# summa-dev/halo2-experiments

Hardware: AMD Instinct MI355X
Metric: BN256 G1 MSM throughput (higher is better)
Workload: dtype u32; 1 GPU; standalone BN256 G1 MSM, 2^24 points per GPU (global 2^24 x 1; BASELINE configs[4] microbench, north-star headline size); points_per_gpu=16777216, global_points=16777216, base_set=fixed-base table (registration default from 2^17 points), window_bits=22, windows=12, parallelism=index-range shards x1, all-gather of 96 B partials (RCCL) + host fold, base_set_bytes=12901679104

## Files before the change

halo2-experiments_amd/csrc/g1.h:

```cpp
#pragma once
#include "ff29.h"

namespace hm {

using Fq = Fe<FqParams>;
using Fr = Fe<FrParams>;

struct G1Aff {
  Fq x, y;
};
struct G1Jac {
  Fq x, y, z;
  bool inf;
};

#define HM_G1_XB 12.0
#define HM_G1_YB 5.0
#define HM_G1_ZB 2.0

#ifdef HM_BOUNDS
inline void g1_check_class(const G1Jac& p, const char* what) {
  HM_CHECK(p.x.lb <= MASK29 && p.y.lb <= MASK29 && p.z.lb <= MASK29, what);
  HM_CHECK(p.x.vb <= HM_G1_XB && p.y.vb <= HM_G1_YB && p.z.vb <= HM_G1_ZB, what);
}
// ... 202 lines not shown
  } else {
    u2 = fe_mul(q.x, acc.zz);
  }
  const Fq pp0 = fe_norm(fe_sub<9, 29>(u2, acc.x));
  if constexpr (!LOCKSTEP) {
    pp = fe_sqr(pp0);
    if (fe_is_zero_mod(pp)) return false;
    s2p = fe_mul(q.y, acc.zzz);
  }
  Fq s2;
  {
    const Fq s2n = fe_sub<3, 29>(fe_zero<FqParams>(), s2p);
#pragma unroll
    for (int i = 0; i < 9; ++i) s2.l[i] = neg ? s2n.l[i] : s2p.l[i];
#ifdef HM_BOUNDS
    s2.vb = s2n.vb; s2.lb = s2n.lb; s2.tb = s2n.tb;
#endif
  }
  const Fq r = fe_norm(fe_sub<4, 29>(s2, acc.y));
  if constexpr (LOCKSTEP) {
    fe_sqr_x2(pp, rr, pp0, r);
    if (fe_is_zero_mod(pp)) return false;
    fe_mul_x3(ppp, qq, zz3, pp0, pp, acc.x, pp, acc.zz, pp);
  } else {
    ppp = fe_mul(pp0, pp);
    qq = fe_mul(acc.x, pp);
    rr = fe_sqr(r);
  }
  const Fq t2 = fe_add(ppp, fe_dbl(qq));
  const Fq x3 = fe_norm(fe_sub<6, 31>(rr, t2));
  const Fq vx = fe_sub<9, 29>(qq, x3);
  const Fq ny = fe_sub<4, 29>(fe_zero<FqParams>(), acc.y);
  if constexpr (LOCKSTEP) {
    fe_mul_mul2(zzz3, y3, acc.zzz, ppp, r, vx, ny, ppp);
  } else {
    y3 = fe_mul2(r, vx, ny, ppp);
    zz3 = fe_mul(acc.zz, pp);
    zzz3 = fe_mul(acc.zzz, ppp);
  }
  acc.x = x3;
  acc.y = y3;
  acc.zz = zz3;
  acc.zzz = zzz3;
  return true;
}

HM_HD G1Xyzz g1x_madd(const G1Xyzz& p, const G1Aff& q, bool neg = false) {
  if (p.inf) return g1x_from_affine(neg ? g1_neg_affine(q) : q);
  G1Xyzz r = p;
  if (g1x_madd_fast(r, q, neg)) return r;
  return g1x_from_jac(g1_madd_nz(g1x_to_jac(p), q, neg));
}

}
```

halo2-experiments_amd/csrc/host_check.cpp:

```cpp
#include <algorithm>
#include <cstring>
#include <utility>
#include <vector>

#include "g1.h"
#include "graph_lower.h"
#include "host_fr.h"
#include "mock_check.h"

namespace hm {
#include "g1_codec.inc"
#include "verify_read.inc"
#include "verify_terms.inc"
#include "poseidon.inc"
#include "range.inc"
#include "keygen.inc"
#include "shplonk.inc"
#include "pairing.inc"
#include "transcript.inc"
}

using namespace hm;

namespace {
// ... 173 lines not shown
}
void hc_g1_double(const uint64_t* pj, int pinf, uint64_t* out, int* out_inf) {
  store_jac(out, out_inf, g1_double(load_jac(pj, pinf)));
}
void hc_g1_chain(const uint64_t* q_aff, int k, int dbl, uint64_t* out, int* out_inf) {
  G1Aff q;
  q.x = load_ext<FqParams>(q_aff);
  q.y = load_ext<FqParams>(q_aff + 4);
  G1Jac acc = g1_identity();
  for (int i = 0; i < k; ++i) acc = g1_madd(acc, q);
  for (int i = 0; i < dbl; ++i) acc = g1_double(acc);
  store_jac(out, out_inf, acc);
}

void hc_g1x_chain(const uint64_t* q_affs, int k, uint64_t signs, uint64_t* out, int* out_inf) {
  G1Xyzz acc = g1x_identity();
  for (int i = 0; i < k; ++i) {
    G1Aff q;
    q.x = load_ext<FqParams>(q_affs + 8 * i);
    q.y = load_ext<FqParams>(q_affs + 8 * i + 4);
    acc = g1x_madd(acc, q, ((signs >> (i & 63)) & 1) != 0);
  }
  store_jac(out, out_inf, g1x_to_jac(acc));
}

int hc_xyzz_bounds_closure(const uint64_t* pj, const uint64_t* q_aff, double* report) {
  G1Jac pjac = load_jac(pj, 0);
  G1Xyzz p = g1x_from_jac(pjac);
  force_bounds(p.x, HM_XYZZ_XB);
  force_bounds(p.y, HM_XYZZ_YB);
  force_bounds(p.zz, 2.0);
  force_bounds(p.zzz, 2.0);
  G1Aff q;
  q.x = load_ext<FqParams>(q_aff);
  q.y = load_ext<FqParams>(q_aff + 4);
  force_bounds(q.x, 2.0);
  force_bounds(q.y, 2.0);
  G1Xyzz r = p;
  if (!g1x_madd_fast(r, q, true)) return 0;
  {
    G1Xyzz rl = p;
    if (!g1x_madd_fast<true>(rl, q, true)) return 0;
    for (int i = 0; i < 9; ++i)
      if (rl.x.l[i] != r.x.l[i] || rl.y.l[i] != r.y.l[i] || rl.zz.l[i] != r.zz.l[i] || rl.zzz.l[i] != r.zzz.l[i]) return 0;
    if (rl.x.vb > HM_XYZZ_XB || rl.y.vb > HM_XYZZ_YB || rl.zz.vb > 2.0 || rl.zzz.vb > 2.0) return 0;
  }
  const G1Jac j = g1x_to_jac(p);
  report[0] = r.x.vb; report[1] = r.y.vb; report[2] = r.zz.vb; report[3] = r.zzz.vb;
  report[4] = j.x.vb; report[5] = j.y.vb; report[6] = j.z.vb;
  int ok = 1;
  if (r.x.vb > HM_XYZZ_XB || r.y.vb > HM_XYZZ_YB || r.zz.vb > 2.0 || r.zzz.vb > 2.0) ok = 0;
  if (j.x.vb > HM_G1_XB || j.y.vb > HM_G1_YB || j.z.vb > HM_G1_ZB) ok = 0;
  return ok;
}

int hc_bounds_closure(const uint64_t* pj, const uint64_t* qj, const uint64_t* q_aff, double* report) {
  G1Jac p = load_jac(pj, 0), q2 = load_jac(qj, 0);
  at_class_max(p);
  at_class_max(q2);
  G1Aff q;
  q.x = load_ext<FqParams>(q_aff);
  q.y = load_ext<FqParams>(q_aff + 4);
  force_bounds(q.x, 2.0);
  force_bounds(q.y, 2.0);
  G1Jac r[3] = {g1_madd_nz(p, q, true), g1_add_nz(p, q2), g1_double_nz(p)};
  int ok = 1;
  for (int i = 0; i < 3; ++i) {
    report[3 * i + 0] = r[i].x.vb;
    report[3 * i + 1] = r[i].y.vb;
    report[3 * i + 2] = r[i].z.vb;
    if (r[i].x.vb > HM_G1_XB || r[i].y.vb > HM_G1_YB || r[i].z.vb > HM_G1_ZB) ok = 0;
    if (r[i].x.lb > MASK29 || r[i].y.lb > MASK29 || r[i].z.lb > MASK29) ok = 0;
  }
  return ok;
}

int hc_graph_bounds_closure(const uint64_t* a_ext, double* report) {
  typedef Fe<FrParams> F;
  F x = load_ext<FrParams>(a_ext);
  const double CAP = 16.0;
  int ok = 1, r = 0;
  F c16 = x, c16b = x, c3 = x, col = x;
  force_bounds(c16, CAP);
  force_bounds(c16b, CAP);
  force_bounds(c3, 3.0);
  force_bounds(col, 6.0);
  F m = fe_mul(c16, c16b);
  report[r++] = m.vb;
  ok &= m.vb <= 3.0;
  F q = fe_sqr(c16);
  ok &= q.vb <= 3.0;
  ok &= fe_mul(col, c16).vb <= 3.0;
  F h8 = x;
  force_bounds(h8, 8.0);
  F s16 = fe_norm(fe_add(h8, h8));
  report[r++] = s16.vb;
  ok &= s16.vb <= CAP;
  F red = fe_reduce_small(fe_norm(fe_add(c16, c16b)));
  ok &= red.vb <= 3.0;
  F dbl = fe_reduce_small(fe_norm(fe_dbl(c16)));
  ok &= dbl.vb <= 3.0;
  F d12 = x;
  force_bounds(d12, 12.0);
  F sub_lazy = fe_norm(fe_sub<4, 29>(d12, c3));
  report[r++] = sub_lazy.vb;
  ok &= sub_lazy.vb <= CAP;
// ... 641 lines not shown
```

halo2-experiments_amd/csrc/msm.hip:

```cpp
#include <hip/hip_runtime.h>

#include <algorithm>
#include <chrono>
#include <cmath>
#include <cstdlib>

#include "hm_internal.h"
#include "host_fq.h"
#include "host_fr.h"
#include "msm_dev.h"

namespace hm {


__global__ void msm_init_counters_kernel(uint32_t* __restrict__ bcnt, size_t nbt, uint32_t* __restrict__ br_count,
                                         uint32_t* __restrict__ khist, uint32_t nkeys, uint32_t* __restrict__ big_count) {
  const size_t i0 = (size_t)blockIdx.x * blockDim.x + threadIdx.x, stride = (size_t)gridDim.x * blockDim.x;
  for (size_t i = i0; i < nbt; i += stride) bcnt[i] = 0;
  if (i0 < nkeys) khist[i0] = 0;
  if (i0 < 4) {
    if (br_count) br_count[i0] = 0;
    big_count[i0] = 0;
  }
}
// ... 1069 lines not shown
    if (rem) {
      const uint32_t key = task_key(rem, L);
      task_bucket[t0 + full] = b;
      task_order[base[key] + atomicAdd(&h[key], 1u)] = t0 + full;
    }
  }
  __syncthreads();
  const uint32_t nh = hot_n < ORDER_HOT ? hot_n : ORDER_HOT;
  for (uint32_t e = 0; e < nh; ++e) {
    const uint32_t b = hot[e][0], t0 = hot[e][1], full = hot[e][2], at = hot[e][3];
    for (uint32_t i = threadIdx.x; i < full; i += ORDER_THREADS) {
      task_bucket[t0 + i] = b;
      task_order[at + i] = t0 + i;
    }
  }
}

#ifndef HM_K3_WAVES
#define HM_K3_WAVES 4
#endif
#define HM_K3_OCC __attribute__((amdgpu_waves_per_eu(HM_K3_WAVES, HM_K3_WAVES)))
__global__ __launch_bounds__(ACC_THREADS) HM_K3_OCC void msm_accumulate_kernel(const uint32_t* __restrict__ sorted,
                                                                     const uint32_t* __restrict__ task_bucket,
                                                                     const uint32_t* __restrict__ task_order,
                                                                     const uint32_t* __restrict__ boff,
                                                                     const uint32_t* __restrict__ bcnt,
                                                                     const uint32_t* __restrict__ toff,
                                                                     const uint32_t* __restrict__ xy,
                                                                     uint32_t* __restrict__ partial,
                                                                     const uint32_t* __restrict__ totals,
                                                                     const uint32_t* __restrict__ pairs, uint32_t L_host) {
  __shared__ uint4 stage[4][ACC_THREADS];
  const uint32_t L = effective_task_len(pairs, L_host);
  const uint32_t lane = threadIdx.x;
  const uint32_t slot = blockIdx.x * ACC_THREADS + lane;
  const uint32_t T = totals[1];
  uint32_t start = 0, end = 0, t = 0;
  if (slot < T) {
    t = task_order[slot];
    const uint32_t b = task_bucket[t];
    const uint32_t k = t - toff[b];
    start = boff[b] + k * L;
    const uint32_t bucket_end = boff[b] + bcnt[b];
    end = start + L < bucket_end ? start + L : bucket_end;
  }
  if (start >= end) return;
  const G1Jac res = accumulate_chain<true>(sorted, xy, start, end, stage, lane);
  store_jac(partial + (size_t)t * PT_WORDS, res);
}


constexpr uint32_t FINALIZE_SERIAL = 8;
constexpr uint32_t FINALIZE_SLICE = 2048;
__global__ __launch_bounds__(ACC_THREADS) void msm_bucket_finalize_kernel(const uint32_t* __restrict__ partial,
                                                                          const uint32_t* __restrict__ toff,
                                                                          uint32_t* __restrict__ bucket, uint32_t NBT,
                                                                          uint32_t* __restrict__ big_count,
                                                                          uint32_t* __restrict__ big_list,
                                                                          uint2* __restrict__ slice_list,
                                                                          const uint32_t* __restrict__ totals) {
  const uint32_t b = blockIdx.x * ACC_THREADS + threadIdx.x;
  if (b >= NBT) return;
  if (totals[2]) {
    store_jac(bucket + (size_t)b * PT_WORDS, g1_identity());
    return;
  }
  const uint32_t lo = toff[b], hi = toff[b + 1];
  if (hi - lo > FINALIZE_SERIAL) {
    big_list[atomicAdd(big_count, 1u)] = b;
    if (hi - lo > FINALIZE_SLICE) {
      const uint32_t nsl = (hi - lo + FINALIZE_SLICE - 1) / FINALIZE_SLICE;
      const uint32_t at = atomicAdd(big_count + 1, nsl);
      for (uint32_t k = 0; k < nsl; ++k) slice_list[at + k] = make_uint2(b, k);
    }
    return;
  }
  G1Jac acc = g1_identity();
  for (uint32_t t = lo; t < hi; ++t) acc = g1_add(acc, load_jac(partial + (size_t)t * PT_WORDS));
  store_jac(bucket + (size_t)b * PT_WORDS, acc);
}

__global__ __launch_bounds__(WIN_THREADS) void msm_bucket_finalize_slices_kernel(uint32_t* __restrict__ partial,
                                                                                 const uint32_t* __restrict__ toff,
                                                                                 const uint32_t* __restrict__ big_count,
                                                                                 const uint2* __restrict__ slice_list) {
  __shared__ uint32_t tree[WIN_THREADS * PT_WORDS];
  const uint32_t count = big_count[1];
  for (uint32_t item = blockIdx.x; item < count; item += gridDim.x) {
    const uint2 e = slice_list[item];
    const uint32_t lo = toff[e.x] + e.y * FINALIZE_SLICE;
    const uint32_t end = toff[e.x + 1], hi = lo + FINALIZE_SLICE < end ? lo + FINALIZE_SLICE : end;
    G1Jac acc = g1_identity();
    for (uint32_t t = lo + threadIdx.x; t < hi; t += WIN_THREADS) acc = g1_add(acc, load_jac(partial + (size_t)t * PT_WORDS));
    const G1Jac r = block_sum_points(tree, acc);
    if (threadIdx.x == 0) store_jac(partial + (size_t)lo * PT_WORDS, r);
    __syncthreads();
  }
}

__global__ __launch_bounds__(WIN_THREADS) void msm_bucket_finalize_big_kernel(const uint32_t* __restrict__ partial,
                                                                              const uint32_t* __restrict__ toff,
                                                                              uint32_t* __restrict__ bucket,
                                                                              const uint32_t* __restrict__ big_count,
                                                                              const uint32_t* __restrict__ big_list) {
  __shared__ uint32_t tree[WIN_THREADS * PT_WORDS];
  const uint32_t count = *big_count;
  for (uint32_t item = blockIdx.x; item < count; item += gridDim.x) {
    const uint32_t b = big_list[item];
    const uint32_t lo = toff[b], hi = toff[b + 1];
    const uint32_t step = hi - lo > FINALIZE_SLICE ? FINALIZE_SLICE : 1u;
    G1Jac acc = g1_identity();
    for (uint32_t t = lo + threadIdx.x * step; t < hi; t += WIN_THREADS * step)
      acc = g1_add(acc, load_jac(partial + (size_t)t * PT_WORDS));
    const G1Jac r = block_sum_points(tree, acc);
    if (threadIdx.x == 0) store_jac(bucket + (size_t)b * PT_WORDS, r);
    __syncthreads();
  }
}

__global__ __launch_bounds__(ACC_THREADS) void msm_reduce_segments_kernel(const uint32_t* __restrict__ bucket,
                                                                          uint32_t* __restrict__ segres, uint32_t W,
                                                                          uint32_t NB, uint32_t NBP, uint32_t SEG,
                                                                          uint32_t nseg) {
  const uint32_t idx = blockIdx.x * ACC_THREADS + threadIdx.x;
  if (idx >= W * nseg) return;
  const uint32_t w = idx / nseg, sgi = idx - w * nseg;
  const uint32_t lo = sgi * SEG + 1;
  const uint32_t hi = lo + SEG - 1 < NB ? lo + SEG - 1 : NB;
  const uint32_t* bw = bucket + (size_t)w * NBP * PT_WORDS;
  G1Jac run = g1_identity(), acc = g1_identity();
  G1Jac cur = hi >= lo ? load_jac(bw + (size_t)hi * PT_WORDS) : g1_identity();
  for (uint32_t b = hi; b >= lo; --b) {
    const G1Jac nxt = b > lo ? load_jac(bw + (size_t)(b - 1) * PT_WORDS) : g1_identity();
    run = g1_add(run, cur);
    acc = g1_add(acc, run);
    cur = nxt;
  }
  uint32_t m = lo - 1;
  if (m != 0 && !run.inf) {
    G1Jac r = g1_identity();
    for (int bit = 31 - __clz(m); bit >= 0; --bit) {
      r = g1_double(r);
      if ((m >> bit) & 1) r = g1_add(r, run);
    }
    acc = g1_add(acc, r);
  }
  store_jac(segres + (size_t)idx * PT_WORDS, acc);
}

#ifndef HM_SUM_PER_LANE
#define HM_SUM_PER_LANE 4
#endif
constexpr uint32_t SUM_SPAN = WIN_THREADS * HM_SUM_PER_LANE;
__global__ __launch_bounds__(WIN_THREADS) void msm_sum_points_kernel(const uint32_t* __restrict__ in, uint32_t count,
                                                                     uint32_t* __restrict__ out, uint32_t out_count) {
  __shared__ uint32_t tree[WIN_THREADS * PT_WORDS];
  const uint32_t w = blockIdx.y, blk = blockIdx.x, t = threadIdx.x;
  const uint32_t* sw = in + (size_t)w * count * PT_WORDS;
  const uint32_t lo = blk * SUM_SPAN, hi = lo + SUM_SPAN < count ? lo + SUM_SPAN : count;
  G1Jac acc = g1_identity();
  for (uint32_t s = lo + t; s < hi; s += WIN_THREADS) acc = g1_add(acc, load_jac(sw + (size_t)s * PT_WORDS));
  const G1Jac r = block_sum_points(tree, acc);
  if (t == 0) store_jac(out + ((size_t)w * out_count + blk) * PT_WORDS, r);
}

__global__ __launch_bounds__(WIN_THREADS) void msm_reduce_rowcol_kernel(const uint32_t* __restrict__ bucket, uint32_t* __restrict__ sums,
                                                                        uint32_t m, uint32_t h) {
  __shared__ uint32_t tree[WIN_THREADS * PT_WORDS];
  const uint32_t M = 1u << m, H = 1u << h, blk = blockIdx.x, t = threadIdx.x;
  bucket += (size_t)blockIdx.y * ((size_t)M * H + 1) * PT_WORDS;
  sums += (size_t)blockIdx.y * ((size_t)M + H) * PT_WORDS;
  const bool row = blk < H;
  const uint32_t count = row ? M : H;
  const uint32_t first = row ? blk * M : blk - H, stride = row ? 1u : M;
  const uint32_t* b1 = bucket + PT_WORDS;
  G1Jac acc = g1_identity();
  if (t < count) {
    G1Jac cur = load_jac(b1 + (size_t)(first + t * stride) * PT_WORDS);
    for (uint32_t e = t; e < count; e += WIN_THREADS) {
      const uint32_t en = e + WIN_THREADS;
      const G1Jac nxt = en < count ? load_jac(b1 + (size_t)(first + en * stride) * PT_WORDS) : g1_identity();
      acc = g1_add(acc, cur);
      cur = nxt;
    }
  }
  const G1Jac r = block_sum_points_upto(tree, acc, count < WIN_THREADS ? count : WIN_THREADS);
  if (t == 0) store_jac(sums + (size_t)blk * PT_WORDS, r);
}

__global__ __launch_bounds__(WIN_THREADS) void msm_reduce_bits_kernel(const uint32_t* __restrict__ sums, uint32_t m, uint32_t h,
                                                                      uint32_t* __restrict__ winres, uint32_t res_stride) {
  __shared__ uint32_t tree[WIN_THREADS * PT_WORDS];
  const uint32_t M = 1u << m, H = 1u << h, p = blockIdx.x, t = threadIdx.x;
  sums += (size_t)blockIdx.y * ((size_t)M + H) * PT_WORDS;
  if (blockIdx.y != 0 && p == 0 && t < 4) (winres - 4)[(size_t)blockIdx.y * res_stride + t] = (winres - 4)[t];
  winres += (size_t)blockIdx.y * res_stride;
  const uint32_t* rows = sums;
  const uint32_t* cols = sums + (size_t)H * PT_WORDS;
  G1Jac acc = g1_identity();
  uint32_t widest = 0;
  if (p < m) {
    const uint32_t half = M >> 1, low = (1u << p) - 1u;
    for (uint32_t i = t; i < half; i += WIN_THREADS) {
      const uint32_t lo = ((i & ~low) << 1) | (1u << p) | (i & low);
      acc = g1_add(acc, load_jac(cols + (size_t)lo * PT_WORDS));
    }
    widest = half;
    if (p == 0) {
      for (uint32_t hi = t; hi < H; hi += WIN_THREADS) acc = g1_add(acc, load_jac(rows + (size_t)hi * PT_WORDS));
      if (H > widest) widest = H;
    }
  } else {
    const uint32_t q = p - m, half = H >> 1, low = (1u << q) - 1u;
    for (uint32_t i = t; i < half; i += WIN_THREADS) {
      const uint32_t hi = ((i & ~low) << 1) | (1u << q) | (i & low);
      acc = g1_add(acc, load_jac(rows + (size_t)hi * PT_WORDS));
    }
    widest = half;
  }
  if (widest > WIN_THREADS) widest = WIN_THREADS;
  if (widest < 1) widest = 1;
  const G1Jac r = block_sum_points_upto(tree, acc, widest);
  if (t == 0) store_window_ext(winres + (size_t)p * 32, r);
}

__global__ void msm_windows_to_ext_kernel(const uint32_t* __restrict__ in, uint32_t W, uint32_t* __restrict__ winres) {
  const uint32_t w = blockIdx.x * blockDim.x + threadIdx.x;
  if (w >= W) return;
  store_window_ext(winres + (size_t)w * 32, load_jac(in + (size_t)w * PT_WORDS));
}

struct G1AffineWords {
  uint32_t w[16];
};
__global__ void g1_fixed_table_kernel(G1AffineWords base_ext, uint32_t* __restrict__ table) {
  const uint32_t w = blockIdx.x * blockDim.x + threadIdx.x;
  if (w >= 64) return;
  uint32_t wx[8], wy[8];
#pragma unroll
  for (int k = 0; k < 8; ++k) { wx[k] = base_ext.w[k]; wy[k] = base_ext.w[8 + k]; }
  G1Aff b;
  b.x = fe_from_ext<FqParams>(wx);
  b.y = fe_from_ext<FqParams>(wy);
  G1Jac p = g1_from_affine(b);
  for (uint32_t k = 0; k < 4 * w; ++k) p = g1_double(p);
  G1Jac acc = p;
  for (uint32_t d = 1; d <= 15; ++d) {
    store_jac(table + ((size_t)w * 15 + (d - 1)) * PT_WORDS, acc);
    acc = g1_add(acc, p);
  }
}

__device__ __forceinline__ Fq fq_inverse(const Fq& a) {
  uint32_t e[9];
#pragma unroll
  for (int i = 0; i < 9; ++i) e[i] = FqParams::MOD[i];
  e[0] -= 2;
  Fq acc = fe_one<FqParams>();
  for (int i = 8; i >= 0; --i) {
    const int top = i == 8 ? 24 : 28;
    for (int bit = top; bit >= 0; --bit) {
      acc = fe_sqr(acc);
      if ((e[i] >> bit) & 1) acc = fe_mul(acc, a);
    }
  }
  return acc;
}

__global__ __launch_bounds__(ACC_THREADS) void msm_precompute_kernel(uint32_t* __restrict__ table,
                                                                     const uint8_t* __restrict__ inf, size_t n, uint32_t c,
                                                                     uint32_t W, uint32_t n_wide) {
  const size_t i = (size_t)blockIdx.x * ACC_THREADS + threadIdx.x;
  if (i >= n) return;
  if (inf[i]) {
    for (uint32_t j = 1; j < W; ++j) {
      uint4* o = reinterpret_cast<uint4*>(table + ((size_t)j * n + i) * 16);
// ... 409 lines not shown
  const uint32_t RW = k4_2d ? c - 1 : SW;
  const uint32_t res_stride = 4 + RW * 32;
  uint32_t ib = ilog2(sn) + ((sn & (sn - 1)) ? 1u : 0u);
  if (ib == 0) ib = 1;
  bool wide_items = false;
  Positional ps{nullptr, 0, 0, 0};
  uint32_t fb = c - 1 < 31 - ib ? c - 1 : 31 - ib;
  if (fb > 15) fb = 15;
#ifndef HM_NO_POSITIONAL
  if (single_set && c >= 14 && c <= 24 && (c - 1) - fb > 10) {
    static const uint32_t cb_first = [] { const char* v = std::getenv("HALO2_MI355X_CB_FIRST"); return (uint32_t)(v && *v ? std::atoi(v) : 9); }();
    for (uint32_t cb_try = cb_first; cb_try <= 12 && ps.nsc == 0; ++cb_try) {
      if (c - 1 < cb_try + 5) break;
      const uint32_t fb_p = c - 1 - cb_try, sbits = 31 - fb_p;
      if (fb_p > 12 || sbits < 16) continue;
      size_t chunk_p = (size_t)1 << 16;
      while ((sn + chunk_p - 1) / chunk_p > 4096 && chunk_p < ((size_t)1 << sbits)) chunk_p <<= 1;
      const size_t nsc = (sn + ((size_t)1 << sbits) - 1) >> sbits;
      if (nsc > PS_MAX_SC || (sn + chunk_p - 1) / chunk_p > 4096) continue;
      ib = sbits;
      fb = fb_p;
      G = (uint32_t)((sn + chunk_p - 1) / chunk_p);
      chunk = chunk_p;
      ps.G = G;
      ps.gpc = (uint32_t)(((size_t)1 << sbits) / chunk_p);
      ps.nsc = (uint32_t)nsc;
    }
  }
#endif
  if (ps.nsc == 0 && fb < 5 && c - 1 > fb) {
    wide_items = true;
    fb = c - 1 < 9 ? c - 1 : 9;
  }
  if (ps.nsc == 0 && sn >= (1u << 15) && (c - 1) - fb < 5) fb = c - 1 > 5 ? c - 1 - 5 : 0;
  const uint32_t cb = (c - 1) - fb, NC = 1u << cb;

  auto align = [](size_t v) { return (v + 255) & ~(size_t)255; };
  size_t off = 0;
  auto carve = [&](size_t bytes) { size_t o = off; off += align(bytes); return o; };
  const size_t o_digits = carve((size_t)W * n * 4 * group);
  const size_t o_chist = carve((size_t)SW * G * NC * 4);
  const size_t o_ctot = carve((size_t)SW * NC * 4);
  const size_t o_cstart = carve(((size_t)SW * NC + 1) * 4);
  const size_t o_tmp = carve(cb ? pairs_max * (wide_items ? 8 : 4) : 4);
  const size_t o_bcnt = carve((size_t)NBT * 4);
  const size_t o_boff = carve((size_t)NBT * 4);
  const size_t o_toff = carve(((size_t)NBT + 1) * 4);
  const size_t o_bsum = carve(((size_t)NBT / SCAN_BLOCK + 2) * 8);
  const size_t o_sorted = carve(pairs_max * 4);
  const size_t o_tb = carve(T_max * 4);
  const size_t o_torder = carve(T_max * 4);
  const size_t o_tkeys = carve(2 * TASK_KEYS * 4);
  const size_t o_partial = carve(T_max * PT_WORDS * 4);
  const size_t o_bucket = carve((size_t)NBT * PT_WORDS * 4);
  const size_t o_seg = carve(k4_2d ? (((size_t)1 << k4_m) + ((size_t)1 << k4_h)) * PT_WORDS * 4 * SW : (size_t)SW * nseg * PT_WORDS * 4);
  const size_t o_seg2 = carve(((size_t)SW * (nseg / SUM_SPAN + 1)) * PT_WORDS * 4);
  const size_t o_res = carve((size_t)(single_set ? group : 1u) * res_stride * 4);
  const size_t o_big = carve(((size_t)NBT + 4) * 4);
  const size_t o_slices = carve((T_max / FINALIZE_SLICE + T_max / (FINALIZE_SERIAL + 1) + 2) * 8);
  BigRegionPlan br;
  {
    const uint64_t mean_region = pairs_max / ((uint64_t)NC * SW) + 1;
    uint64_t slice = (mean_region + P2_TILE - 1) / P2_TILE * P2_TILE;
    if (slice < 4 * (uint64_t)P2_TILE) slice = 4 * (uint64_t)P2_TILE;
    br.slice = (uint32_t)slice;
    br.big = (uint32_t)(4 * slice);
    br.capacity = (uint32_t)(pairs_max / slice + pairs_max / br.big + 2);
  }
  const bool coop_sort = cb != 0 && (fb <= 11 || (ps.nsc != 0 && fb <= 12));
  const size_t o_brlist = carve(coop_sort ? (size_t)br.capacity * 8 : 8);
  const size_t o_brcount = carve(16);
  const size_t o_gcur = carve(coop_sort ? (size_t)NBT * 4 : 4);
  uint8_t* ws = (uint8_t*)sl.ws.ensure(off);
  if (!ws) return hm_fail(HM_ERR_HIP, "msm: workspace allocation failed");
  int32_t* d_digits = (int32_t*)(ws + o_digits);
  uint32_t* d_chist = (uint32_t*)(ws + o_chist);
  uint32_t* d_ctot = (uint32_t*)(ws + o_ctot);
  uint32_t* d_cstart = (uint32_t*)(ws + o_cstart);
  void* d_tmp = (void*)(ws + o_tmp);
  uint32_t* d_bcnt = (uint32_t*)(ws + o_bcnt);
  uint32_t* d_boff = (uint32_t*)(ws + o_boff);
  uint32_t* d_toff = (uint32_t*)(ws + o_toff);
  uint32_t* d_bsum = (uint32_t*)(ws + o_bsum);
  uint32_t* d_sorted = (uint32_t*)(ws + o_sorted);
  uint32_t* d_tb = (uint32_t*)(ws + o_tb);
  uint32_t* d_torder = (uint32_t*)(ws + o_torder);
  uint32_t* d_khist = (uint32_t*)(ws + o_tkeys);
  uint32_t* d_kcursor = d_khist + TASK_KEYS;
  uint32_t* d_partial = (uint32_t*)(ws + o_partial);
  uint32_t* d_bucket = (uint32_t*)(ws + o_bucket);
  uint32_t* d_seg = (uint32_t*)(ws + o_seg);
  uint32_t* d_seg2 = (uint32_t*)(ws + o_seg2);
  uint32_t* d_tot = (uint32_t*)(ws + o_res);
  uint32_t* d_win = d_tot + 4;
  uint32_t* d_big_count = (uint32_t*)(ws + o_big);
  uint32_t* d_big_list = d_big_count + 4;
  uint2* d_slices = (uint2*)(ws + o_slices);
  br.list = (uint2*)(ws + o_brlist);
  br.count = (uint32_t*)(ws + o_brcount);
  br.gcursor = (uint32_t*)(ws + o_gcur);
  if (!coop_sort) br.big = 0xffffffffu;

  if (!ctx.msm_attr_set) {
    const int lds_max = 32768 * 4;
    HM_HIP_CHECK(hipFuncSetAttribute(reinterpret_cast<const void*>(msm_part2_hist_kernel<true, uint32_t, false>),
                                     hipFuncAttributeMaxDynamicSharedMemorySize, lds_max));
    HM_HIP_CHECK(hipFuncSetAttribute(reinterpret_cast<const void*>(msm_part2_hist_kernel<false, uint32_t, false>),
                                     hipFuncAttributeMaxDynamicSharedMemorySize, lds_max));
// ... 68 lines not shown
                         cb ? br.count : (uint32_t*)nullptr, d_khist, TASK_KEYS, d_big_count);
      HM_HIP_CHECK(hipGetLastError());
    }
    const int rc = wide_items
                       ? launch_sort<uint64_t>(d_digits, d_chist, d_ctot, d_cstart, d_tmp, d_bcnt, sn, chunk, G, SW, fb, ib, cb,
                                               NC, NBP, br, stream)
                       : launch_sort<uint32_t>(d_digits, d_chist, d_ctot, d_cstart, d_tmp, d_bcnt, sn, chunk, G, SW, fb, ib, cb,
                                               NC, NBP, br, stream);
    if (rc != HM_OK) return rc;
  }
  const uint32_t* d_pairs = cb ? (const uint32_t*)(d_cstart + (size_t)SW * NC) : (const uint32_t*)nullptr;
  {
    const uint32_t nblocks = (NBT + SCAN_BLOCK - 1) / SCAN_BLOCK;
    hipLaunchKernelGGL(msm_scan_partial_kernel, dim3(nblocks), dim3(SCAN_THREADS), 0, stream, (const uint32_t*)d_bcnt,
                       d_bsum, NBT, d_pairs, L);
    hipLaunchKernelGGL(msm_scan_blocksums_kernel, dim3(1), dim3(SCAN_THREADS), 0, stream, d_bsum, nblocks, d_tot,
                       (uint32_t)std::min<uint64_t>(T_max, 0xffffffffull));
    hipLaunchKernelGGL(msm_scan_final_kernel, dim3(nblocks), dim3(SCAN_THREADS), 0, stream, (const uint32_t*)d_bcnt,
                       (const uint32_t*)d_bsum, d_boff, d_toff, (const uint32_t*)d_tot, NBT, d_pairs, L,
                       coop_sort ? br.gcursor : (uint32_t*)nullptr);
    HM_HIP_CHECK(hipGetLastError());
  }
  {
    ps.chist = d_chist;
    const int rc = wide_items ? launch_sort_scatter<uint64_t>(d_digits, d_cstart, d_tmp, d_boff, d_sorted, sn, SW, fb, ib, cb, NC,
                                                              NBP, NBT, br, ps, stream)
                              : launch_sort_scatter<uint32_t>(d_digits, d_cstart, d_tmp, d_boff, d_sorted, sn, SW, fb, ib, cb, NC,
                                                              NBP, NBT, br, ps, stream);
    if (rc != HM_OK) return rc;
  }
  if (pairs_max < (1u << 19)) {
    hipLaunchKernelGGL(msm_task_fill_kernel, dim3((NBT + 255) / 256), dim3(256), 0, stream, (const uint32_t*)d_toff, d_tb, d_torder,
                       NBT, (const uint32_t*)d_tot);
  } else {
    const uint32_t og = (NBT + ORDER_THREADS * ORDER_ITEMS - 1) / (ORDER_THREADS * ORDER_ITEMS);
    hipLaunchKernelGGL(msm_task_hist_kernel, dim3(og), dim3(ORDER_THREADS), 0, stream, (const uint32_t*)d_bcnt, NBT,
                       d_pairs, L, d_khist);
    hipLaunchKernelGGL(msm_task_keyscan_kernel, dim3(1), dim3(ORDER_THREADS), 0, stream, (const uint32_t*)d_khist, d_kcursor);
    hipLaunchKernelGGL(msm_task_order_kernel, dim3(og), dim3(ORDER_THREADS), 0, stream, (const uint32_t*)d_bcnt,
                       (const uint32_t*)d_toff, NBT, d_pairs, L, d_kcursor, d_tb, d_torder, (const uint32_t*)d_tot);
  }
  HM_HIP_CHECK(hipGetLastError());
  if (pt) HM_HIP_CHECK(hipEventRecord(ev[2], stream));

  if (pt) HM_HIP_CHECK(hipEventRecord(ev[5], stream));
  {
    const uint64_t t_grid = T_max;
    hipLaunchKernelGGL(msm_accumulate_kernel, dim3((uint32_t)((t_grid + ACC_THREADS - 1) / ACC_THREADS)), dim3(ACC_THREADS), 0,
                       stream, (const uint32_t*)d_sorted, (const uint32_t*)d_tb, (const uint32_t*)d_torder, (const uint32_t*)d_boff,
                       (const uint32_t*)d_bcnt, (const uint32_t*)d_toff, d_xy, d_partial, (const uint32_t*)d_tot, d_pairs, L);
    HM_HIP_CHECK(hipGetLastError());
  }
  if (pt) HM_HIP_CHECK(hipEventRecord(ev[6], stream));
  hipLaunchKernelGGL(msm_bucket_finalize_kernel, dim3((NBT + ACC_THREADS - 1) / ACC_THREADS), dim3(ACC_THREADS), 0, stream,
                     (const uint32_t*)d_partial, (const uint32_t*)d_toff, d_bucket, NBT, d_big_count, d_big_list, d_slices,
                     (const uint32_t*)d_tot);
  HM_HIP_CHECK(hipGetLastError());
  {
    uint32_t slice_grid = (uint32_t)(T_max / FINALIZE_SLICE + 1);
    if (slice_grid > 2048) slice_grid = 2048;
    hipLaunchKernelGGL(msm_bucket_finalize_slices_kernel, dim3(slice_grid), dim3(WIN_THREADS), 0, stream, d_partial,
                       (const uint32_t*)d_toff, (const uint32_t*)d_big_count, (const uint2*)d_slices);
    uint32_t big_grid = (uint32_t)(T_max / (FINALIZE_SERIAL + 1) + 1);
    if (big_grid > 2048) big_grid = 2048;
    hipLaunchKernelGGL(msm_bucket_finalize_big_kernel, dim3(big_grid), dim3(WIN_THREADS), 0, stream,
                       (const uint32_t*)d_partial, (const uint32_t*)d_toff, d_bucket, (const uint32_t*)d_big_count,
                       (const uint32_t*)d_big_list);
    HM_HIP_CHECK(hipGetLastError());
  }
  if (pt) HM_HIP_CHECK(hipEventRecord(ev[3], stream));

  if (k4_2d) {
    hipLaunchKernelGGL(msm_reduce_rowcol_kernel, dim3((1u << k4_m) + (1u << k4_h), SW), dim3(WIN_THREADS), 0, stream,
                       (const uint32_t*)d_bucket, d_seg, k4_m, k4_h);
    hipLaunchKernelGGL(msm_reduce_bits_kernel, dim3(RW, SW), dim3(WIN_THREADS), 0, stream, (const uint32_t*)d_seg, k4_m, k4_h, d_win,
                       res_stride);
    HM_HIP_CHECK(hipGetLastError());
  } else {
  hipLaunchKernelGGL(msm_reduce_segments_kernel, dim3((SW * nseg + ACC_THREADS - 1) / ACC_THREADS), dim3(ACC_THREADS), 0,
                     stream, (const uint32_t*)d_bucket, d_seg, SW, NB, NBP, SEG, nseg);
  HM_HIP_CHECK(hipGetLastError());
  {
    uint32_t* cur = d_seg;
    uint32_t* nxt = d_seg2;
    uint32_t count = nseg;
    while (count > 1) {
      const uint32_t out_count = (count + SUM_SPAN - 1) / SUM_SPAN;
      hipLaunchKernelGGL(msm_sum_points_kernel, dim3(out_count, SW), dim3(WIN_THREADS), 0, stream, (const uint32_t*)cur, count, nxt,
                         out_count);
      HM_HIP_CHECK(hipGetLastError());
      uint32_t* t = cur; cur = nxt; nxt = t;
      count = out_count;
    }
    hipLaunchKernelGGL(msm_windows_to_ext_kernel, dim3((SW + 63) / 64), dim3(64), 0, stream, (const uint32_t*)cur, SW, d_win);
    HM_HIP_CHECK(hipGetLastError());
  }
  }
  if (RW > 128) return hm_fail(HM_ERR_INTERNAL, "msm: more than 128 windows");
  HM_HIP_CHECK(hipMemcpyAsync(sl.totals(), d_tot, (size_t)(single_set ? group : 1u) * res_stride * 4, hipMemcpyDeviceToHost, stream));
  HM_HIP_CHECK(hipEventRecord(ev[4], stream));
  return HM_OK;
}

int msm_enqueue(DeviceCtx& ctx, int slot, const uint32_t* d_scalars_ext, const uint32_t* d_xy, const uint8_t* d_inf, size_t n,
                uint32_t precomp_c, hipStream_t stream) {
  MsmSlot& sl = ctx.msm_slots[slot];
  sl.n = n;
  sl.stream = stream;
  sl.group = 1;
  if (n == 0) return HM_OK;
  return msm_issue(ctx, slot, &d_scalars_ext, 1, d_xy, d_inf, n, precomp_c, stream);
}

uint32_t msm_table_group_max(size_t n, uint32_t precomp_c) {
  static const uint32_t want = [] {
    const char* v = std::getenv("HALO2_MI355X_GROUP_DENSE");
    const int g = v && *v ? std::atoi(v) : 8;
    return (uint32_t)(g < 1 ? 1 : g > HM_MSM_GROUP ? HM_MSM_GROUP : g);
  }();
  static const bool k4_chain_only = [] { const char* v = std::getenv("HALO2_MI355X_K4_CHAIN"); return v && *v == '1'; }();
  if (precomp_c < 6 || n == 0 || n >= ((size_t)1 << 19) || k4_chain_only || msm_small_applies(n, precomp_c, true)) return 1;
  const uint64_t per = (uint64_t)n * ((255 + precomp_c - 1) / precomp_c);
  uint32_t g = want;
  while (g > 1 && per * g >= (1ull << 31)) --g;
  while (g > 1 && per * g * 4 > ((uint64_t)3 << 30)) --g;
  return g;
// ... 223 lines not shown
```

halo2-experiments_amd/csrc/msm_dev.h:

```cpp
#pragma once
#include <hip/hip_runtime.h>

#include "g1.h"

namespace hm {

constexpr int PT_WORDS = 28;

__device__ __forceinline__ G1Jac load_jac(const uint32_t* p) {
  const uint4* q = reinterpret_cast<const uint4*>(p);
  uint32_t w[PT_WORDS];
#pragma unroll
  for (int i = 0; i < 7; ++i) {
    const uint4 v = q[i];
    w[4 * i] = v.x; w[4 * i + 1] = v.y; w[4 * i + 2] = v.z; w[4 * i + 3] = v.w;
  }
  G1Jac r;
#pragma unroll
  for (int i = 0; i < 9; ++i) {
    r.x.l[i] = w[i];
    r.y.l[i] = w[9 + i];
    r.z.l[i] = w[18 + i];
  }
  r.inf = w[27] != 0;
  return r;
}
__device__ __forceinline__ void store_jac(uint32_t* p, const G1Jac& a) {
  uint32_t w[PT_WORDS];
#pragma unroll
  for (int i = 0; i < 9; ++i) {
    w[i] = a.x.l[i];
    w[9 + i] = a.y.l[i];
    w[18 + i] = a.z.l[i];
  }
  w[27] = a.inf ? 1u : 0u;
  uint4* q = reinterpret_cast<uint4*>(p);
#pragma unroll
  for (int i = 0; i < 7; ++i) q[i] = make_uint4(w[4 * i], w[4 * i + 1], w[4 * i + 2], w[4 * i + 3]);
}

__device__ __forceinline__ G1Aff load_base(const uint32_t* xy, uint32_t idx) {
  const uint4* q = reinterpret_cast<const uint4*>(xy + (size_t)idx * 16);
  const uint4 a = q[0], b = q[1], c = q[2], d = q[3];
  const uint32_t wx[8] = {a.x, a.y, a.z, a.w, b.x, b.y, b.z, b.w};
  const uint32_t wy[8] = {c.x, c.y, c.z, c.w, d.x, d.y, d.z, d.w};
  G1Aff r;
  r.x = fe_unpack<FqParams>(wx);
  r.y = fe_unpack<FqParams>(wy);
  return r;
}

constexpr int ACC_THREADS = 64;

typedef __attribute__((address_space(3))) void hm_lds_void;
typedef __attribute__((address_space(1))) const void hm_gbl_void;

__device__ __forceinline__ void stage_base_async(const uint32_t* xy, uint32_t idx, uint4 (*stage)[ACC_THREADS]) {
  const uint4* src = reinterpret_cast<const uint4*>(xy + (size_t)idx * 16);
#pragma unroll
  for (int k = 0; k < 4; ++k)
    __builtin_amdgcn_global_load_lds((hm_gbl_void*)(src + k), (hm_lds_void*)&stage[k][0], 16, 0, 0);
}

template <bool LOCKSTEP = false>
__device__ __forceinline__ G1Jac accumulate_chain(const uint32_t* __restrict__ sorted, const uint32_t* __restrict__ xy,
                                                  uint32_t start, uint32_t end, uint4 (*stage)[ACC_THREADS], uint32_t lane) {
  uint32_t v_cur = sorted[start];
  G1Xyzz acc;
  {
    const G1Aff q0 = load_base(xy, v_cur & 0x7fffffffu);
    acc = g1x_from_affine((v_cur >> 31) ? g1_neg_affine(q0) : q0);
  }
  uint32_t p = start + 1, v_next = 0;
  if (p < end) {
    v_cur = sorted[p];
    stage_base_async(xy, v_cur & 0x7fffffffu, stage);
    if (p + 1 < end) v_next = sorted[p + 1];
  }
  bool general = false;
  for (; p < end; ++p) {
    asm volatile("s_waitcnt vmcnt(0)" ::: "memory");
    const uint4 a = stage[0][lane], b4 = stage[1][lane], c4 = stage[2][lane], d4 = stage[3][lane];
    asm volatile("s_waitcnt lgkmcnt(0)" ::: "memory");
    const bool neg = (v_cur >> 31) != 0;
    if (p + 1 < end) {
      v_cur = v_next;
      stage_base_async(xy, v_cur & 0x7fffffffu, stage);
      if (p + 2 < end) v_next = sorted[p + 2];
    }
    const uint32_t wx[8] = {a.x, a.y, a.z, a.w, b4.x, b4.y, b4.z, b4.w};
    const uint32_t wy[8] = {c4.x, c4.y, c4.z, c4.w, d4.x, d4.y, d4.z, d4.w};
// ... 14 lines not shown
    }
  }
  return res;
}

constexpr int WIN_THREADS = 256;
__device__ __forceinline__ G1Jac block_sum_points(uint32_t* tree, G1Jac acc) {
  const uint32_t t = threadIdx.x;
  store_jac(tree + t * PT_WORDS, acc);
  __syncthreads();
  for (uint32_t off = WIN_THREADS / 2; off > 0; off >>= 1) {
    if (t < off) {
      const G1Jac a = load_jac(tree + t * PT_WORDS), b = load_jac(tree + (t + off) * PT_WORDS);
      store_jac(tree + t * PT_WORDS, g1_add(a, b));
    }
    __syncthreads();
  }
  return load_jac(tree);
}


__device__ __forceinline__ uint32_t lds_inc(uint32_t* cnt, uint32_t bin) {
#ifndef HM_NO_AGG
  const uint32_t v = (uint32_t)__builtin_amdgcn_readfirstlane((int)bin);
  const uint64_t active = __ballot(1);
  if (__ballot(bin == v) == active) {
    const uint32_t lane = __builtin_amdgcn_mbcnt_hi(~0u, __builtin_amdgcn_mbcnt_lo(~0u, 0u));
    const uint32_t before = (uint32_t)__popcll(active & ((1ull << lane) - 1ull));
    uint32_t base = 0;
    if (before == 0) base = atomicAdd(&cnt[v], (uint32_t)__popcll(active));
    base = (uint32_t)__builtin_amdgcn_readfirstlane((int)base);
    return base + before;
  }
#endif
  return atomicAdd(&cnt[bin], 1u);
}

__device__ __forceinline__ G1Jac block_sum_points_upto(uint32_t* tree, G1Jac acc, uint32_t count) {
  const uint32_t t = threadIdx.x;
  uint32_t top = 1;
  while (top < count) top <<= 1;
  if (t < top) store_jac(tree + t * PT_WORDS, acc);
  __syncthreads();
  for (uint32_t off = top / 2; off > 0; off >>= 1) {
    if (t < off) {
      const G1Jac a = load_jac(tree + t * PT_WORDS), b = load_jac(tree + (t + off) * PT_WORDS);
      store_jac(tree + t * PT_WORDS, g1_add(a, b));
    }
    __syncthreads();
  }
  return load_jac(tree);
}

__device__ __forceinline__ void store_window_ext(uint32_t* o, const G1Jac& r) {
  uint32_t wx[8], wy[8], wz[8];
  if (r.inf) {
#pragma unroll
    for (int k = 0; k < 8; ++k) wx[k] = wy[k] = wz[k] = 0;
  } else {
    fe_to_ext(wx, r.x);
    fe_to_ext(wy, r.y);
    fe_to_ext(wz, r.z);
  }
#pragma unroll
  for (int k = 0; k < 8; ++k) {
    o[k] = wx[k];
    o[8 + k] = wy[k];
    o[16 + k] = wz[k];
  }
  o[24] = r.inf ? 1u : 0u;
}

}
```

Baseline: 985.9 million points/s.

## Use XYZZ coordinates for bucket storage and 2D row/column bucket reduction

Adds a general XYZZ+XYZZ addition (with an optional lockstep multiply variant) and switches the 2D bucket-reduction path (finalize output, row/column sums, bit reductions, tree sums) from Jacobian to XYZZ points. XYZZ addition needs fewer field multiplies than Jacobian addition, which is meant to cut reduction cost. It also shrinks the row/column kernel block from 256 to 64 threads. In exchange each stored point grows from 28 to 40 words, adding memory traffic and LDS use, and the finalize step pays an extra Jacobian-to-XYZZ conversion per bucket.

```diff
diff --git a/halo2-experiments_amd/csrc/g1.h b/halo2-experiments_amd/csrc/g1.h
--- a/halo2-experiments_amd/csrc/g1.h
+++ b/halo2-experiments_amd/csrc/g1.h
@@ -278,4 +278,60 @@
   return g1x_from_jac(g1_madd_nz(g1x_to_jac(p), q, neg));
 }
 
-}
+template <bool LOCKSTEP = false>
+HM_HD bool g1x_add_fast(G1Xyzz& acc, const G1Xyzz& q) {
+  HM_G1_CHECK(acc, "g1x_add_fast accumulator outside class");
+  HM_G1_CHECK(q, "g1x_add_fast operand outside class");
+  Fq u1, u2, s1, s2, zz12, zzz12, pp, rr, ppp, qq, zz3, zzz3, y3;
+  if constexpr (LOCKSTEP) {
+    fe_mul_x3(u1, u2, zz12, acc.x, q.zz, q.x, acc.zz, acc.zz, q.zz);
+    fe_mul_x3(s1, s2, zzz12, acc.y, q.zzz, q.y, acc.zzz, acc.zzz, q.zzz);
+  } else {
+    u1 = fe_mul(acc.x, q.zz);
+    u2 = fe_mul(q.x, acc.zz);
+  }
+  const Fq pp0 = fe_norm(fe_sub<3, 29>(u2, u1));
+  if constexpr (!LOCKSTEP) {
+    pp = fe_sqr(pp0);
+    if (fe_is_zero_mod(pp)) return false;
+    s1 = fe_mul(acc.y, q.zzz);
+    s2 = fe_mul(q.y, acc.zzz);
+  }
+  const Fq r = fe_norm(fe_sub<3, 29>(s2, s1));
+  if constexpr (LOCKSTEP) {
+    fe_sqr_x2(pp, rr, pp0, r);
+    if (fe_is_zero_mod(pp)) return false;
+    fe_mul_x3(ppp, qq, zz3, pp0, pp, u1, pp, zz12, pp);
+  } else {
+    ppp = fe_mul(pp0, pp);
+    qq = fe_mul(u1, pp);
+    rr = fe_sqr(r);
+  }
+  const Fq t2 = fe_add(ppp, fe_dbl(qq));
+  const Fq x3 = fe_norm(fe_sub<6, 31>(rr, t2));
+  const Fq vx = fe_sub<9, 29>(qq, x3);
+  const Fq ns1 = fe_sub<3, 29>(fe_zero<FqParams>(), s1);
+  if constexpr (LOCKSTEP) {
+    fe_mul_mul2(zzz3, y3, zzz12, ppp, r, vx, ns1, ppp);
+  } else {
+    y3 = fe_mul2(r, vx, ns1, ppp);
+    zz3 = fe_mul(fe_mul(acc.zz, q.zz), pp);
+    zzz3 = fe_mul(fe_mul(acc.zzz, q.zzz), ppp);
+  }
+  acc.x = x3;
+  acc.y = y3;
+  acc.zz = zz3;
+  acc.zzz = zzz3;
+  return true;
+}
+
+template <bool LOCKSTEP = false>
+HM_HD G1Xyzz g1x_add(const G1Xyzz& p, const G1Xyzz& q) {
+  if (p.inf) return q;
+  if (q.inf) return p;
+  G1Xyzz r = p;
+  if (g1x_add_fast<LOCKSTEP>(r, q)) return r;
+  return g1x_from_jac(g1_add_nz(g1x_to_jac(p), g1x_to_jac(q)));
+}
+
+}
diff --git a/halo2-experiments_amd/csrc/host_check.cpp b/halo2-experiments_amd/csrc/host_check.cpp
--- a/halo2-experiments_amd/csrc/host_check.cpp
+++ b/halo2-experiments_amd/csrc/host_check.cpp
@@ -249,6 +249,26 @@
   if (r.x.vb > HM_XYZZ_XB || r.y.vb > HM_XYZZ_YB || r.zz.vb > 2.0 || r.zzz.vb > 2.0) ok = 0;
   if (j.x.vb > HM_G1_XB || j.y.vb > HM_G1_YB || j.z.vb > HM_G1_ZB) ok = 0;
   return ok;
+}
+
+int hc_xyzz_add_bounds_closure(const uint64_t* pj, const uint64_t* qj, double* report) {
+  G1Xyzz p = g1x_from_jac(load_jac(pj, 0)), q = g1x_from_jac(load_jac(qj, 0));
+  for (G1Xyzz* a : {&p, &q}) {
+    force_bounds(a->x, HM_XYZZ_XB);
+    force_bounds(a->y, HM_XYZZ_YB);
+    force_bounds(a->zz, 2.0);
+    force_bounds(a->zzz, 2.0);
+  }
+  G1Xyzz r = p, rl = p;
+  if (!g1x_add_fast(r, q) || !g1x_add_fast<true>(rl, q)) return 0;
+  for (int i = 0; i < 9; ++i)
+    if (rl.x.l[i] != r.x.l[i] || rl.y.l[i] != r.y.l[i] || rl.zz.l[i] != r.zz.l[i] || rl.zzz.l[i] != r.zzz.l[i]) return 0;
+  report[0] = r.x.vb; report[1] = r.y.vb; report[2] = r.zz.vb; report[3] = r.zzz.vb;
+  for (const G1Xyzz* a : {&r, &rl}) {
+    if (a->x.vb > HM_XYZZ_XB || a->y.vb > HM_XYZZ_YB || a->zz.vb > 2.0 || a->zzz.vb > 2.0) return 0;
+    if (a->x.lb > MASK29 || a->y.lb > MASK29 || a->zz.lb > MASK29 || a->zzz.lb > MASK29) return 0;
+  }
+  return 1;
 }
 
 int hc_bounds_closure(const uint64_t* pj, const uint64_t* qj, const uint64_t* q_aff, double* report) {
diff --git a/halo2-experiments_amd/csrc/msm.hip b/halo2-experiments_amd/csrc/msm.hip
--- a/halo2-experiments_amd/csrc/msm.hip
+++ b/halo2-experiments_amd/csrc/msm.hip
@@ -1145,6 +1145,7 @@
 
 constexpr uint32_t FINALIZE_SERIAL = 8;
 constexpr uint32_t FINALIZE_SLICE = 2048;
+template <bool XYZZ>
 __global__ __launch_bounds__(ACC_THREADS) void msm_bucket_finalize_kernel(const uint32_t* __restrict__ partial,
                                                                           const uint32_t* __restrict__ toff,
                                                                           uint32_t* __restrict__ bucket, uint32_t NBT,
@@ -1155,10 +1156,17 @@
   const uint32_t b = blockIdx.x * ACC_THREADS + threadIdx.x;
   if (b >= NBT) return;
   if (totals[2]) {
-    store_jac(bucket + (size_t)b * PT_WORDS, g1_identity());
+    if constexpr (XYZZ) store_xyzz(bucket + (size_t)b * XP_WORDS, g1x_identity());
+    else store_jac(bucket + (size_t)b * PT_WORDS, g1_identity());
     return;
   }
   const uint32_t lo = toff[b], hi = toff[b + 1];
+  if constexpr (XYZZ) {
+    if (hi == lo) {
+      store_xyzz(bucket + (size_t)b * XP_WORDS, g1x_identity());
+      return;
+    }
+  }
   if (hi - lo > FINALIZE_SERIAL) {
     big_list[atomicAdd(big_count, 1u)] = b;
     if (hi - lo > FINALIZE_SLICE) {
@@ -1170,7 +1178,8 @@
   }
   G1Jac acc = g1_identity();
   for (uint32_t t = lo; t < hi; ++t) acc = g1_add(acc, load_jac(partial + (size_t)t * PT_WORDS));
-  store_jac(bucket + (size_t)b * PT_WORDS, acc);
+  if constexpr (XYZZ) store_xyzz(bucket + (size_t)b * XP_WORDS, g1x_from_jac(acc));
+  else store_jac(bucket + (size_t)b * PT_WORDS, acc);
 }
 
 __global__ __launch_bounds__(WIN_THREADS) void msm_bucket_finalize_slices_kernel(uint32_t* __restrict__ partial,
@@ -1191,6 +1200,7 @@
   }
 }
 
+template <bool XYZZ>
 __global__ __launch_bounds__(WIN_THREADS) void msm_bucket_finalize_big_kernel(const uint32_t* __restrict__ partial,
                                                                               const uint32_t* __restrict__ toff,
                                                                               uint32_t* __restrict__ bucket,
@@ -1206,7 +1216,10 @@
     for (uint32_t t = lo + threadIdx.x * step; t < hi; t += WIN_THREADS * step)
       acc = g1_add(acc, load_jac(partial + (size_t)t * PT_WORDS));
     const G1Jac r = block_sum_points(tree, acc);
-    if (threadIdx.x == 0) store_jac(bucket + (size_t)b * PT_WORDS, r);
+    if (threadIdx.x == 0) {
+      if constexpr (XYZZ) store_xyzz(bucket + (size_t)b * XP_WORDS, g1x_from_jac(r));
+      else store_jac(bucket + (size_t)b * PT_WORDS, r);
+    }
     __syncthreads();
   }
 }
@@ -1257,64 +1270,77 @@
   if (t == 0) store_jac(out + ((size_t)w * out_count + blk) * PT_WORDS, r);
 }
 
-__global__ __launch_bounds__(WIN_THREADS) void msm_reduce_rowcol_kernel(const uint32_t* __restrict__ bucket, uint32_t* __restrict__ sums,
-                                                                        uint32_t m, uint32_t h) {
-  __shared__ uint32_t tree[WIN_THREADS * PT_WORDS];
+#ifndef HM_RC_THREADS
+#define HM_RC_THREADS 64
+#endif
+constexpr uint32_t RC_THREADS = HM_RC_THREADS;
+__global__ __launch_bounds__(RC_THREADS) void msm_reduce_rowcol_kernel(const uint32_t* __restrict__ bucket, uint32_t* __restrict__ sums,
+                                                                       uint32_t m, uint32_t h) {
+  __shared__ uint32_t tree[RC_THREADS * XP_WORDS];
   const uint32_t M = 1u << m, H = 1u << h, blk = blockIdx.x, t = threadIdx.x;
-  bucket += (size_t)blockIdx.y * ((size_t)M * H + 1) * PT_WORDS;
-  sums += (size_t)blockIdx.y * ((size_t)M + H) * PT_WORDS;
+  bucket += (size_t)blockIdx.y * ((size_t)M * H + 1) * XP_WORDS;
+  sums += (size_t)blockIdx.y * ((size_t)M + H) * XP_WORDS;
   const bool row = blk < H;
   const uint32_t count = row ? M : H;
   const uint32_t first = row ? blk * M : blk - H, stride = row ? 1u : M;
-  const uint32_t* b1 = bucket + PT_WORDS;
-  G1Jac acc = g1_identity();
+  const uint32_t* b1 = bucket + XP_WORDS;
+  G1Xyzz acc = g1x_identity();
   if (t < count) {
-    G1Jac cur = load_jac(b1 + (size_t)(first + t * stride) * PT_WORDS);
-    for (uint32_t e = t; e < count; e += WIN_THREADS) {
-      const uint32_t en = e + WIN_THREADS;
-      const G1Jac nxt = en < count ? load_jac(b1 + (size_t)(first + en * stride) * PT_WORDS) : g1_identity();
-      acc = g1_add(acc, cur);
+    uint32_t e = t;
+    bool general = false;
+    G1Xyzz cur = load_xyzz(b1 + (size_t)(first + t * stride) * XP_WORDS);
+    for (; e < count; e += RC_THREADS) {
+      const uint32_t en = e + RC_THREADS;
+      const G1Xyzz nxt = en < count ? load_xyzz(b1 + (size_t)(first + en * stride) * XP_WORDS) : g1x_identity();
+      if (acc.inf) {
+        acc = cur;
+      } else if (!cur.inf && !g1x_add_fast<XADD_LOCKSTEP>(acc, cur)) {
+        general = true;
+        break;
+      }
       cur = nxt;
     }
-  }
-  const G1Jac r = block_sum_points_upto(tree, acc, count < WIN_THREADS ? count : WIN_THREADS);
-  if (t == 0) store_jac(sums + (size_t)blk * PT_WORDS, r);
+    if (general)
+      for (; e < count; e += RC_THREADS) acc = g1x_add<XADD_LOCKSTEP>(acc, load_xyzz(b1 + (size_t)(first + e * stride) * XP_WORDS));
+  }
+  const G1Xyzz r = block_sum_xyzz_upto(tree, acc, count < RC_THREADS ? count : RC_THREADS);
+  if (t == 0) store_xyzz(sums + (size_t)blk * XP_WORDS, r);
 }
 
 __global__ __launch_bounds__(WIN_THREADS) void msm_reduce_bits_kernel(const uint32_t* __restrict__ sums, uint32_t m, uint32_t h,
                                                                       uint32_t* __restrict__ winres, uint32_t res_stride) {
-  __shared__ uint32_t tree[WIN_THREADS * PT_WORDS];
+  __shared__ uint32_t tree[WIN_THREADS * XP_WORDS];
   const uint32_t M = 1u << m, H = 1u << h, p = blockIdx.x, t = threadIdx.x;
-  sums += (size_t)blockIdx.y * ((size_t)M + H) * PT_WORDS;
+  sums += (size_t)blockIdx.y * ((size_t)M + H) * XP_WORDS;
   if (blockIdx.y != 0 && p == 0 && t < 4) (winres - 4)[(size_t)blockIdx.y * res_stride + t] = (winres - 4)[t];
   winres += (size_t)blockIdx.y * res_stride;
   const uint32_t* rows = sums;
-  const uint32_t* cols = sums + (size_t)H * PT_WORDS;
-  G1Jac acc = g1_identity();
+  const uint32_t* cols = sums + (size_t)H * XP_WORDS;
+  G1Xyzz acc = g1x_identity();
   uint32_t widest = 0;
   if (p < m) {
     const uint32_t half = M >> 1, low = (1u << p) - 1u;
     for (uint32_t i = t; i < half; i += WIN_THREADS) {
       const uint32_t lo = ((i & ~low) << 1) | (1u << p) | (i & low);
-      acc = g1_add(acc, load_jac(cols + (size_t)lo * PT_WORDS));
+      acc = g1x_add<XADD_LOCKSTEP>(acc, load_xyzz(cols + (size_t)lo * XP_WORDS));
     }
     widest = half;
     if (p == 0) {
-      for (uint32_t hi = t; hi < H; hi += WIN_THREADS) acc = g1_add(acc, load_jac(rows + (size_t)hi * PT_WORDS));
+      for (uint32_t hi = t; hi < H; hi += WIN_THREADS) acc = g1x_add<XADD_LOCKSTEP>(acc, load_xyzz(rows + (size_t)hi * XP_WORDS));
       if (H > widest) widest = H;
     }
   } else {
     const uint32_t q = p - m, half = H >> 1, low = (1u << q) - 1u;
     for (uint32_t i = t; i < half; i += WIN_THREADS) {
       const uint32_t hi = ((i & ~low) << 1) | (1u << q) | (i & low);
-      acc = g1_add(acc, load_jac(rows + (size_t)hi * PT_WORDS));
+      acc = g1x_add<XADD_LOCKSTEP>(acc, load_xyzz(rows + (size_t)hi * XP_WORDS));
     }
     widest = half;
   }
   if (widest > WIN_THREADS) widest = WIN_THREADS;
   if (widest < 1) widest = 1;
-  const G1Jac r = block_sum_points_upto(tree, acc, widest);
-  if (t == 0) store_window_ext(winres + (size_t)p * 32, r);
+  const G1Xyzz r = block_sum_xyzz_upto(tree, acc, widest);
+  if (t == 0) store_window_ext(winres + (size_t)p * 32, g1x_to_jac(r));
 }
 
 __global__ void msm_windows_to_ext_kernel(const uint32_t* __restrict__ in, uint32_t W, uint32_t* __restrict__ winres) {
@@ -1830,8 +1856,8 @@
   const size_t o_torder = carve(T_max * 4);
   const size_t o_tkeys = carve(2 * TASK_KEYS * 4);
   const size_t o_partial = carve(T_max * PT_WORDS * 4);
-  const size_t o_bucket = carve((size_t)NBT * PT_WORDS * 4);
-  const size_t o_seg = carve(k4_2d ? (((size_t)1 << k4_m) + ((size_t)1 << k4_h)) * PT_WORDS * 4 * SW : (size_t)SW * nseg * PT_WORDS * 4);
+  const size_t o_bucket = carve((size_t)NBT * (k4_2d ? XP_WORDS : PT_WORDS) * 4);
+  const size_t o_seg = carve(k4_2d ? (((size_t)1 << k4_m) + ((size_t)1 << k4_h)) * XP_WORDS * 4 * SW : (size_t)SW * nseg * PT_WORDS * 4);
   const size_t o_seg2 = carve(((size_t)SW * (nseg / SUM_SPAN + 1)) * PT_WORDS * 4);
   const size_t o_res = carve((size_t)(single_set ? group : 1u) * res_stride * 4);
   const size_t o_big = carve(((size_t)NBT + 4) * 4);
@@ -2006,9 +2032,12 @@
     HM_HIP_CHECK(hipGetLastError());
   }
   if (pt) HM_HIP_CHECK(hipEventRecord(ev[6], stream));
-  hipLaunchKernelGGL(msm_bucket_finalize_kernel, dim3((NBT + ACC_THREADS - 1) / ACC_THREADS), dim3(ACC_THREADS), 0, stream,
-                     (const uint32_t*)d_partial, (const uint32_t*)d_toff, d_bucket, NBT, d_big_count, d_big_list, d_slices,
-                     (const uint32_t*)d_tot);
+  {
+    const dim3 fin_grid((NBT + ACC_THREADS - 1) / ACC_THREADS);
+    auto finalize = k4_2d ? msm_bucket_finalize_kernel<true> : msm_bucket_finalize_kernel<false>;
+    hipLaunchKernelGGL(finalize, fin_grid, dim3(ACC_THREADS), 0, stream, (const uint32_t*)d_partial, (const uint32_t*)d_toff, d_bucket,
+                       NBT, d_big_count, d_big_list, d_slices, (const uint32_t*)d_tot);
+  }
   HM_HIP_CHECK(hipGetLastError());
   {
     uint32_t slice_grid = (uint32_t)(T_max / FINALIZE_SLICE + 1);
@@ -2017,15 +2046,15 @@
                        (const uint32_t*)d_toff, (const uint32_t*)d_big_count, (const uint2*)d_slices);
     uint32_t big_grid = (uint32_t)(T_max / (FINALIZE_SERIAL + 1) + 1);
     if (big_grid > 2048) big_grid = 2048;
-    hipLaunchKernelGGL(msm_bucket_finalize_big_kernel, dim3(big_grid), dim3(WIN_THREADS), 0, stream,
-                       (const uint32_t*)d_partial, (const uint32_t*)d_toff, d_bucket, (const uint32_t*)d_big_count,
+    hipLaunchKernelGGL(k4_2d ? msm_bucket_finalize_big_kernel<true> : msm_bucket_finalize_big_kernel<false>, dim3(big_grid),
+                       dim3(WIN_THREADS), 0, stream, (const uint32_t*)d_partial, (const uint32_t*)d_toff, d_bucket, (const uint32_t*)d_big_count,
                        (const uint32_t*)d_big_list);
     HM_HIP_CHECK(hipGetLastError());
   }
   if (pt) HM_HIP_CHECK(hipEventRecord(ev[3], stream));
 
   if (k4_2d) {
-    hipLaunchKernelGGL(msm_reduce_rowcol_kernel, dim3((1u << k4_m) + (1u << k4_h), SW), dim3(WIN_THREADS), 0, stream,
+    hipLaunchKernelGGL(msm_reduce_rowcol_kernel, dim3((1u << k4_m) + (1u << k4_h), SW), dim3(RC_THREADS), 0, stream,
                        (const uint32_t*)d_bucket, d_seg, k4_m, k4_h);
     hipLaunchKernelGGL(msm_reduce_bits_kernel, dim3(RW, SW), dim3(WIN_THREADS), 0, stream, (const uint32_t*)d_seg, k4_m, k4_h, d_win,
                        res_stride);
diff --git a/halo2-experiments_amd/csrc/msm_dev.h b/halo2-experiments_amd/csrc/msm_dev.h
--- a/halo2-experiments_amd/csrc/msm_dev.h
+++ b/halo2-experiments_amd/csrc/msm_dev.h
@@ -37,6 +37,43 @@
   uint4* q = reinterpret_cast<uint4*>(p);
 #pragma unroll
   for (int i = 0; i < 7; ++i) q[i] = make_uint4(w[4 * i], w[4 * i + 1], w[4 * i + 2], w[4 * i + 3]);
+}
+
+constexpr int XP_WORDS = 40;
+
+__device__ __forceinline__ G1Xyzz load_xyzz(const uint32_t* p) {
+  const uint4* q = reinterpret_cast<const uint4*>(p);
+  uint32_t w[XP_WORDS];
+#pragma unroll
+  for (int i = 0; i < 10; ++i) {
+    const uint4 v = q[i];
+    w[4 * i] = v.x; w[4 * i + 1] = v.y; w[4 * i + 2] = v.z; w[4 * i + 3] = v.w;
+  }
+  G1Xyzz r;
+#pragma unroll
+  for (int i = 0; i < 9; ++i) {
+    r.x.l[i] = w[i];
+    r.y.l[i] = w[9 + i];
+    r.zz.l[i] = w[18 + i];
+    r.zzz.l[i] = w[27 + i];
+  }
+  r.inf = w[36] != 0;
+  return r;
+}
+__device__ __forceinline__ void store_xyzz(uint32_t* p, const G1Xyzz& a) {
+  uint32_t w[XP_WORDS];
+#pragma unroll
+  for (int i = 0; i < 9; ++i) {
+    w[i] = a.x.l[i];
+    w[9 + i] = a.y.l[i];
+    w[18 + i] = a.zz.l[i];
+    w[27 + i] = a.zzz.l[i];
+  }
+  w[36] = a.inf ? 1u : 0u;
+  w[37] = w[38] = w[39] = 0u;
+  uint4* q = reinterpret_cast<uint4*>(p);
+#pragma unroll
+  for (int i = 0; i < 10; ++i) q[i] = make_uint4(w[4 * i], w[4 * i + 1], w[4 * i + 2], w[4 * i + 3]);
 }
 
 __device__ __forceinline__ G1Aff load_base(const uint32_t* xy, uint32_t idx) {
@@ -157,6 +194,26 @@
   return load_jac(tree);
 }
 
+#ifndef HM_XADD_LOCKSTEP
+#define HM_XADD_LOCKSTEP 0
+#endif
+constexpr bool XADD_LOCKSTEP = HM_XADD_LOCKSTEP != 0;
+__device__ __forceinline__ G1Xyzz block_sum_xyzz_upto(uint32_t* tree, const G1Xyzz& acc, uint32_t count) {
+  const uint32_t t = threadIdx.x;
+  uint32_t top = 1;
+  while (top < count) top <<= 1;
+  if (t < top) store_xyzz(tree + t * XP_WORDS, acc);
+  __syncthreads();
+  for (uint32_t off = top / 2; off > 0; off >>= 1) {
+    if (t < off) {
+      const G1Xyzz a = load_xyzz(tree + t * XP_WORDS), b = load_xyzz(tree + (t + off) * XP_WORDS);
+      store_xyzz(tree + t * XP_WORDS, g1x_add<XADD_LOCKSTEP>(a, b));
+    }
+    __syncthreads();
+  }
+  return load_xyzz(tree);
+}
+
 __device__ __forceinline__ void store_window_ext(uint32_t* o, const G1Jac& r) {
   uint32_t wx[8], wy[8], wz[8];
   if (r.inf) {
```

After: 986.8 million points/s, median of 6. About the same (+0.1%).
